# fritzsedlazeck/Sniffles

Hardware: AMD Instinct MI355X
Metric: SV-signatures clustered/sec (clustering + calling + QC + genotype + INS consensus) (higher is better)
Workload: dtype int32/f64

## Files before the change

sniffles_amd/csrc/snf_fused.h:

```cpp
#pragma once
#include "snf_stage_final.h"
#include "snf_stage_cluster.h"
#include "snf_stage_call.h"

namespace snf {

template <int K>
SNF_D void block_exscan256(const unsigned long long (&val)[K], unsigned long long (&excl)[K], unsigned long long (&tot)[K],
                           unsigned long long* lds) {
  const int tid = threadIdx.x, lane = tid & 63, wid = tid >> 6;
  unsigned long long incl[K];
#pragma unroll
  for (int k = 0; k < K; k++) {
    unsigned long long x = val[k];
#pragma unroll
    for (int d = 1; d < 64; d <<= 1) { const unsigned long long y = __shfl_up(x, d, 64); if (lane >= d) x += y; }
    incl[k] = x;
    if (lane == 63) lds[wid * K + k] = x;
  }
  __syncthreads();
#pragma unroll
  for (int k = 0; k < K; k++) {
    unsigned long long base = 0, all = 0;
#pragma unroll
// ... 119 lines not shown
  __global__ void __launch_bounds__(256) name(const View v, int64_t n) {      \
    __shared__ unsigned long long lds[8];                                     \
    const int64_t p = (int64_t)blockIdx.x * 256 + threadIdx.x;

__global__ void __launch_bounds__(256) z0_init(const View v, int64_t n) {
  const int64_t i = (int64_t)blockIdx.x * 256 + threadIdx.x;
  const int64_t T = v.T, G = 8 * T + 8;
  if (i < (int64_t)(sizeof(Counts) / 8)) {
    unsigned long long c0 = 0;
    if (v.win_ready && i == (int64_t)(offsetof(Counts, n_valid) / 8)) c0 = (unsigned long long)v.win_n_valid;
    if (v.win_ready && i == (int64_t)(offsetof(Counts, n_occ) / 8)) c0 = (unsigned long long)v.win_n_occ;
    ((unsigned long long*)v.cnt)[i] = c0;
  }
  if (i <= T) { v.t_cov_sum[i] = 0; v.t_status[i] = 0; }
  if (i <= T + 1) v.t_call_off[i] = 0;
  if (i < G) { v.grp_first_bin[i] = -1; v.grp_seed_lo[i] = -1; v.grp_seed_hi[i] = -1; v.grp_dirty[i] = 0; }
  if (i < TS_SLOTS * v.super_stride) v.tile_super[i] = 0;
  if (i < v.tile_stride) {
    v.tile_sums[(int64_t)TS_REFINED * v.tile_stride + i] = 0; v.tile_sums[(int64_t)TS_CALLS * v.tile_stride + i] = 0;
  }
  if (i == 0) *v.chain_epoch += 1u;
  if (v.wave_path && i < 3 * 64 * 16) v.big_cnt[i] = 0;
  if (v.wave_path && i < 3 * 64 * 16) v.d2cnt[i] = 0;
  if (i == 0 && v.NS > 0) {
    const int64_t N = v.NS;
    v.headflag[N] = 0; v.eligflag[N] = 0; v.fN[N] = 0; v.fL[N] = 0; v.runflag[N] = 0; v.clflag[N] = 0; v.rcflag[N] = 0; v.cdflag[N] = 0;
  }
}

SNF_FUSED_HEAD(a0k_keep)
  if (p < n) a0_keep_body(p, v);
  unsigned long long val[1] = {p < n ? (unsigned long long)v.pf_keep[p] : 0ull};
  tile_publish<1>(v, TS_KEEP, val, lds);
}
SNF_FUSED_HEAD(a0k_compact)
  unsigned long long val[1] = {p < n ? (unsigned long long)v.pf_keep[p] : 0ull}, off[1];
  tile_scan<1>(v, TS_KEEP, val, off, lds);
  if (p < n) {
    v.pf_scan[p] = (uint32_t)off[0];
    if (p == n - 1) v.cnt->n_kept = (int64_t)(off[0] + val[0]);
    a0_emit(p, v);
  }
}
SNF_FUSED_HEAD(a2k_heads)
  if (p < n) { a2_heads_body(p, v); v.rcflag[p] = 0; }
  unsigned long long val[1] = {p < n ? (unsigned long long)v.headflag[p] : 0ull};
// ... 201 lines not shown
```

sniffles_amd/csrc/snf_knobs.h:

```cpp
#pragma once
#include <climits>
#include <cstdlib>
#include <cstring>
#include <string>

namespace snf {

constexpr int KNOB_UNSET = INT_MIN;
inline bool env_set(const char* name) { return getenv(name) != nullptr; }
inline int env_int(const char* name, int unset) { const char* e = getenv(name); return e ? atoi(e) : unset; }
inline int env_pos(const char* name, int other) { const int v = env_int(name, 0); return v > 0 ? v : other; }
inline bool env_on(const char* name) { return env_int(name, 0) != 0; }
inline bool env_is(const char* name, const char* value) { const char* e = getenv(name); return e && strcmp(e, value) == 0; }
inline std::string env_str(const char* name) { const char* e = getenv(name); return e ? e : ""; }

struct BatchKnobs {
  bool wave_path = !env_set("SNF_NO_WAVE");
  bool fuse = !env_set("SNF_NO_FUSE");
  bool sort64 = env_set("SNF_SORT64");
  bool prefilter = !env_set("SNF_NO_PREFILTER");
  bool pf_spread = env_int("SNF_PF_SPREAD", 0) == 1;
  bool winfront = !env_set("SNF_NO_WINFRONT");
  int win_bits = env_int("SNF_WIN_BITS", 0);
  int win_bits_max = [] { const int v = env_int("SNF_WIN_BITS_MAX", 10); return v >= 6 && v <= 12 ? v : 10; }();
  bool w4_split = env_on("SNF_W4_SPLIT");
  bool pool_slices = !env_set("SNF_NO_POOL_SLICES");
  int fuse_copy = env_set("SNF_FUSE_COPY") ? env_on("SNF_FUSE_COPY") : -1;
  bool merge_reread = env_on("SNF_MERGE_REREAD");
  int run_gap = env_int("SNF_RUN_GAP", KNOB_UNSET);
  int chain = env_set("SNF_CHAIN") ? env_on("SNF_CHAIN") : env_set("SNF_NO_CHAIN") ? 0 : -1;
  int graph = env_set("SNF_GRAPH") ? env_on("SNF_GRAPH") : env_set("SNF_NO_GRAPH") ? 0 : -1;
  int heavy_n = env_int("SNF_HEAVY_N", 24);
  int e1_batch = env_int("SNF_E1_BATCH", 64);
  bool big_stage = !env_set("SNF_NO_BIG_STAGE");
  bool cov_exact = env_set("SNF_COV_EXACT");
  bool d4_thread = env_is("SNF_D4", "thread");
  bool d1_groups = !env_set("SNF_NO_D1_GROUPS");
  bool d2_groups = !env_set("SNF_NO_D2_GROUPS");
  bool d2_mid = env_set("SNF_D2_MID");
  bool rn_defer = !env_set("SNF_NO_RN_DEFER");
  bool rn_fuse = !env_set("SNF_NO_RN_FUSE");
  int grid_mult = env_int("SNF_GRID_MULT", 2);
  int grid_div = env_pos("SNF_GRID_DIV", 1);
  int occ_d2 = env_int("SNF_OCC_D2", 5);
  int occ_e1 = env_int("SNF_OCC_E1", 5);
  int occ_s = env_int("SNF_OCC_S", 5);
  int cons_nw = env_int("SNF_CONS_NW", 1);
  int cons_large_nw = env_int("SNF_CONS_LARGE_NW", 4);
  int cons_grid_mult = env_int("SNF_CONS_GRID_MULT", KNOB_UNSET);
  int cons_small_grid = env_pos("SNF_CONS_SMALL_GRID", 65536);
// ... 63 lines not shown
```

sniffles_amd/csrc/snf_lib.hip:

```cpp
#include "snf_stage_final.h"
#include "snf_wave_refine.h"
#include "snf_wave_cons.h"
#include "snf_fused.h"
#include "snf_stage_window.h"
#include "snf_stage_out.h"
#include "snf_wave_call.h"
#include "snf_wave_call_g.h"
#include "snf_wave_refine_g.h"
#include "snf_ctx.h"

#include <rocprim/device/device_radix_sort.hpp>
#include <rocprim/device/device_scan.hpp>

#include <fcntl.h>
#include <sys/file.h>
#include <unistd.h>

#include <atomic>
#include <map>
#include <tuple>
#include <cmath>
#include <ctime>
#include <memory>
#include <mutex>
// ... 887 lines not shown
    v.ws_seeds = dalloc<uint32_t>(b, nblk); v.ws_nf = dalloc<uint32_t>(b, nblk); v.ws_nl = dalloc<uint32_t>(b, nblk);
    v.whead = dalloc<uint64_t>(b, N1); v.whead2 = dalloc<uint64_t>(b, N1);
    dzero(b, v.wcnt, W1 * 4); dzero(b, v.wfill, W1 * 4);
  }
  uint32_t** u32s[] = {&v.headflag, &v.headscan, &v.eligflag, &v.eligscan, &v.fN, &v.pN, &v.fL, &v.pL, &v.runflag, &v.runscan,
                       &v.clflag, &v.clscan, &v.rcflag, &v.rcscan, &v.cdflag, &v.cdscan, &v.rnf, &v.rnp};
  for (auto pp : u32s) *pp = dalloc<uint32_t>(b, N1);
  v.seqnull = dalloc<uint8_t>(b, N); v.bin_lo = dalloc<int32_t>(b, N1); v.bin_key = dalloc<uint64_t>(b, N);
  v.bin_hap = dalloc<uint16_t>(b, 3 * (size_t)N); v.bin_elig = dalloc<uint8_t>(b, N);
  v.grp_first_bin = dalloc<int32_t>(b, 8 * (size_t)T + 8);
  v.L = dalloc<uint32_t>(b, N); v.LL = dalloc<uint32_t>(b, N); v.Lrec = dalloc<LeadRec>(b, N1); v.chdr = dalloc<ClusterHdr>(b, N1);
  int32_t** i32s[] = {&v.seed_bin, &v.seed_lo, &v.seed_hi, &v.seedL_lo, &v.seedL_hi, &v.seed_start, &v.seed_grp, &v.c_last, &v.c_end,
                      &v.nxt, &v.prv, &v.run_first, &v.run_last_head, &v.cl_head, &v.w0, &v.w1, &v.w2, &v.w3, &v.w4, &v.w5, &v.w6, &v.w7,
                      &v.F_orig, &v.F_svlen, &v.F_seq_len, &v.FI, &v.F_lpos, &v.rc_n_s, &v.rc_cl_s, &v.rc_lo, &v.rc_n, &v.rc_cluster};
  for (auto pp : i32s) *pp = dalloc<int32_t>(b, N1);
  double** f64s[] = {&v.s_mean0, &v.s_stdev0, &v.c_mean, &v.c_stdev, &v.run_b_stdev, &v.run_b_absmean};
  for (auto pp : f64s) *pp = dalloc<double>(b, N1);
  uint8_t** u8s[] = {&v.s_repeat0, &v.c_repeat, &v.run_b_repeat, &v.F_sel, &v.rc_keeplong_s, &v.rc_keeplong};
  for (auto pp : u8s) *pp = dalloc<uint8_t>(b, N1);
  v.c_ms = dalloc<ClusterSums>(b, N1);
  v.grp_dirty = dalloc<int32_t>(b, 8 * (size_t)T + 8); v.grp_seed_lo = dalloc<int32_t>(b, 8 * (size_t)T + 8);
  v.grp_seed_hi = dalloc<int32_t>(b, 8 * (size_t)T + 8);
  v.F_seq_off = dalloc<int64_t>(b, N1);
  v.fcopy = dalloc<FuseDesc>(b, N1); dzero(b, v.fcopy, N1 * sizeof(FuseDesc));
  v.cand = dalloc<snf_call_t>(b, N1); v.candx = dalloc<CallX>(b, N1);
  v.calls = dalloc<snf_call_t>(b, N1); v.callx = dalloc<CallX>(b, N1);
  v.rnames = dalloc<uint32_t>(b, 2 * (size_t)N + 1);
  const auto& lut = build_gt_lut(b->cfg);
  v.gt_lut = upload_vec(b, lut);
  v.cons_call = dalloc<int32_t>(b, N1);
  v.stripes = dalloc<unsigned long long>(b, 4 * 64 * 16);
  v.tile_stride = (int64_t)((N1 > (size_t)win_slots_max + 1 ? N1 : (size_t)win_slots_max + 1) / 256 + 2); v.tile_sums = dalloc<unsigned long long>(b, (size_t)v.tile_stride * TS_SLOTS);
  v.super_stride = v.tile_stride / 64 + 2; v.tile_super = dalloc<unsigned long long>(b, (size_t)v.super_stride * TS_SLOTS);
  v.chain_stride = v.tile_stride; v.chain = dalloc<unsigned long long>(b, (size_t)v.chain_stride * TS_SLOTS * 2);
  v.chain_ticket = dalloc<uint32_t>(b, TS_SLOTS + 2); v.chain_epoch = v.chain_ticket + TS_SLOTS;
  dzero(b, v.chain, (size_t)v.chain_stride * TS_SLOTS * 16); dzero(b, v.chain_ticket, (TS_SLOTS + 2) * 4);
  const bool small_batch = N <= 400000;
  v.chain_on = b->k.chain >= 0 ? b->k.chain : (small_batch ? 1 : 0);
  b->graph_mode = (b->k.graph >= 0 ? b->k.graph != 0 : small_batch) ? 2 : 0;
  v.fuse_defer = v.wave_path && (b->k.fuse_copy >= 0 ? b->k.fuse_copy != 0 : b->graph_mode == 0) ? 1 : 0;
  v.big_cap = (int64_t)(N1 / 64 + 2); v.big_cnt = dalloc<uint32_t>(b, 3 * 64 * 16); v.big_list = dalloc<int32_t>(b, (size_t)(3 * 64 * v.big_cap));
  v.big_wave = v.wave_path;
  { const int hn = b->k.heavy_n; v.heavy_n = hn > 8 && hn < 64 ? hn : 0; }
  v.d1_push = v.wave_path && b->k.d1_groups ? 1 : 0;
  v.d2_push = v.wave_path && b->k.d2_groups ? (b->k.d2_mid ? 2 : 1) : 0;
  { const int eb = b->k.e1_batch; v.e1_batch = (eb == 2 || eb == 4 || eb == 8 || eb == 16 || eb == 32) ? eb : 64; }
  v.stage_cap = b->k.big_stage ? 1 : 0;
// ... 287 lines not shown
  const int64_t n_blk = (N + 63) / 64;
  const bool split = b->k.w4_split && b->win_cap > 64 && b->h_n_big64 > 0 && b->h_n_big64 * 8 < n_blk;
  {
    Scope* sc = b->time_all ? new Scope(b, "w4s_segment", 0) : nullptr;
    if (split) {
      v.w4_mode = 1;
      hipLaunchKernelGGL(w4s_segment<64>, dim3((unsigned)n_blk), dim3(64), 0, b->cur, v, (int64_t)0);
      v.w4_mode = 2;
      if (b->win_cap == 256) hipLaunchKernelGGL(w4s_segment<256>, dim3((unsigned)b->h_n_big64), dim3(64), 0, b->cur, v, (int64_t)0);
      else hipLaunchKernelGGL(w4s_segment<SNF_WIN_MAXCAP>, dim3((unsigned)b->h_n_big64), dim3(64), 0, b->cur, v, (int64_t)0);
      v.w4_mode = 0;
    }
    else if (b->win_cap == 64) hipLaunchKernelGGL(w4s_segment<64>, dim3((unsigned)n_blk), dim3(64), 0, b->cur, v, (int64_t)0);
    else if (b->win_cap == 256) hipLaunchKernelGGL(w4s_segment<256>, dim3((unsigned)n_blk), dim3(64), 0, b->cur, v, (int64_t)0);
    else hipLaunchKernelGGL(w4s_segment<SNF_WIN_MAXCAP>, dim3((unsigned)n_blk), dim3(64), 0, b->cur, v, (int64_t)0);
    delete sc;
    SNF_HIP(hipGetLastError());
  }
  if (v.chain_on) CHAIN(w5c_offsets, n_blk);
  else { FUSED(w5a_sums, n_blk); FUSED(w5b_offsets, n_blk); }
  LAUNCH_Q(w6t_emit, v, N, 0);
}

void enqueue_fuse_copy(snf_batch_impl* b, hipEvent_t after) {
  View& v = b->v;
  if (!after) { SNF_HIP(hipEventRecord(b->ev_refined, b->stream)); after = b->ev_refined; }
  SNF_HIP(hipStreamWaitEvent(b->stream2, after, 0));
  hipStream_t prev = b->cur; b->cur = b->stream2;
  { Scope _s(b, "d1c_fusecopy", 0);
    int64_t grid = (v.NS + 63) / 64; if (grid > 2048) grid = 2048;
    hipLaunchKernelGGL(d1c_fusecopy, dim3((unsigned)grid), dim3(64), 0, b->cur, v, (int64_t)0);
    SNF_HIP(hipGetLastError()); }
  b->cur = prev;
  SNF_HIP(hipEventRecord(b->ev_fcopy, b->stream2));
  b->fcopy_open = true;
}

void run_call_candidates(snf_batch_impl* b) {
  SNF_TRACE("snf_batch_call_candidates (enqueue)");
  b->pass_idle = false;
  View& v = b->v;
  int T = v.T;
  const int64_t N = v.NS;
  b->reads_ready = true; b->cov_avg_ready = true; b->finalized = false;
  begin_pass_timing(b);
  pass_begins(b);
  join_open_candidates(b);
  b->chain_slot = -1;
  if (process_knobs().chain_gate && !b->capturing) {
    DevicePacing& P = pacing_of(b);
    std::lock_guard<std::mutex> g(P.pace_mu);
    const unsigned long long my = P.chain_seq++;
    hipEvent_t& mine = P.chain_ev[my & 1]; hipEvent_t prev = P.chain_ev[(my + 1) & 1];
    if (!mine) SNF_HIP(hipEventCreateWithFlags(&mine, hipEventDisableTiming));
    b->chain_slot = (int)(my & 1);
    if (prev && P.passes_in_flight.load() > 1) SNF_HIP(hipStreamWaitEvent(b->stream, prev, 0));
  }
  v.rn_defer = ((v.out_mode & SNF_OUT_EXECUTE) && !v.cfg.no_qc && b->k.rn_defer && b->k.fuse && N <= ((int64_t)1 << 25)) ? 1 : 0;
  b->rn_state = v.rn_defer ? 1 : 0;
  if (b->k.timeline) SNF_HIP(hipEventRecord(b->ev_base, b->stream));
  enqueue_pass_init(b);
  if (v.wave_path && !b->fused) dzero(b, v.big_cnt, sizeof(uint32_t) * 3 * 64 * 16);
  if (v.wave_path && !b->fused) dzero(b, v.d2cnt, sizeof(uint32_t) * 3 * 64 * 16);
  b->finalize_runs = 0;
  fork_mark(b);
  if (b->k.readprep == 0) enqueue_read_prep(b);
  const bool front = v.front && b->fused && N > 0;
  if (front) enqueue_window_front(b); else enqueue_keys(b);
  if (N > 0) {
    if (!b->fused) {
      uint32_t* tails[] = {v.headflag, v.eligflag, v.fN, v.fL, v.runflag, v.clflag, v.rcflag, v.cdflag};
      for (auto p : tails) dzero(b, p + N, sizeof(uint32_t));
    }
    if (!front) {
    if (v.key32) prim_sort_pairs<uint32_t>(b, (uint32_t*)v.key_in, (uint32_t*)v.key_out, v.val_in, v.val_out, N, v.key_nbits + 1, "sort_lead_keys");
    else prim_sort_pairs<uint64_t>(b, v.key_in, v.key_out, v.val_in, v.val_out, N, v.key_nbits + 1, "sort_lead_keys");
    }
    if (b->fused) {
    if (!front) {
    FUSED(a2k_heads, N);
    FUSED(a3k_bins, N);
    { Scope _s(b, "a4_binstats", N * 16); FUSED(a4k_binstats, N); }
    FUSED(a5k_leadflags, N);
    { Scope _s(b, "a6_scatter", N * 16); FUSED(a6k_scatter, N); }
    FUSED(a7k_seeds, N);
    }
// ... 478 lines not shown
  if (ok) ok = hipGraphInstantiate(&exec, graph, nullptr, nullptr, 0) == hipSuccess && exec != nullptr;
  if (!ok) {
    (void)hipGetLastError();
    if (graph) (void)hipGraphDestroy(graph);
    b->graph_failed = true;
    if (v.prof) fprintf(stderr, "[SNF_PROF] pass graph: capture failed, passes stay eager\n");
    run_call_candidates(b); run_finalize(b);
    return;
  }
  g.graph = graph; g.exec = exec; g.rn_state = b->rn_state; g.rn_defer = v.rn_defer; g.cap_out = b->hb_out.cap; g.cap_alt = b->hb_alt.cap;
  if (v.prof) { size_t nn = 0; (void)hipGraphGetNodes(graph, nullptr, &nn); fprintf(stderr, "[SNF_PROF] pass graph: captured (%zu nodes)\n", nn); }
  SNF_HIP(hipGraphLaunch(g.exec, b->stream));
}
void destroy_graphs(snf_batch_impl* b) {
  for (auto& kv : b->graphs) { if (kv.second.exec) (void)hipGraphExecDestroy(kv.second.exec); if (kv.second.graph) (void)hipGraphDestroy(kv.second.graph); }
  b->graphs.clear();
}

void collect_timings(snf_batch_impl* b) {
  b->timings.clear();
#ifdef SNF_ITRACE
  if (b->k.prof && b->v.itrace) {
    static const char* nm[SNF_IT_SLOTS] = {"w1_hist", "w3_scatter", "w4s_segment", "w6t_emit", "d1g_refine", "d1w_refine", "d2g_call", "d2w_call", "e3b_offsets",
                                           "e1w_finalize", "cons SMALL", "cons LARGE", "d4s_coverage", "f4w_emit", "cons ROWS", ""};
    std::vector<uint32_t> h((size_t)SNF_IT_SLOTS * SNF_IT_CAP * 2);
    (void)hipMemcpy(h.data(), b->v.itrace, h.size() * 4, hipMemcpyDeviceToHost);
    (void)hipMemset(b->v.itrace, 0, h.size() * 4);
    for (int k = 0; k < SNF_IT_SLOTS; k++) {
      struct E { uint32_t t0, dur, wg; };
      std::vector<E> es;
      for (int64_t i = 0; i < SNF_IT_CAP; i++) { const uint32_t* o = &h[2 * ((size_t)k * SNF_IT_CAP + i)]; if (o[1] & 0x80000000u) es.push_back({o[0], o[1] & 0x7fffffffu, (uint32_t)i}); }
      if (es.empty()) continue;
      uint32_t base = es[0].t0;
      for (auto& e : es) if ((int32_t)(e.t0 - base) < 0) base = e.t0;
      uint32_t span = 0; double sum = 0;
      for (auto& e : es) { e.t0 -= base; span = std::max(span, e.t0 + e.dur); sum += e.dur; }
      std::vector<uint32_t> d; for (auto& e : es) d.push_back(e.dur);
      std::sort(d.begin(), d.end());
      auto pc = [&](double q) { return d[(size_t)(q * (d.size() - 1))] * 0.01; };
      fprintf(stderr, "[SNF_ITRACE] %-13s %6zu workgroups, span %7.1f us, sum %9.1f us = %6.0f in flight on average; duration us p50 %.1f p90 %.1f p99 %.1f max %.1f; in flight at 12 points:",
              nm[k], es.size(), span * 0.01, sum * 0.01, sum / (span ? span : 1), pc(0.5), pc(0.9), pc(0.99), pc(1.0));
      for (int q = 0; q < 12; q++) { const uint32_t t = (uint32_t)((uint64_t)span * (2 * q + 1) / 24); int act = 0; for (auto& e : es) act += e.t0 <= t && t < e.t0 + e.dur; fprintf(stderr, " %d", act); }
      std::sort(es.begin(), es.end(), [](const E& a, const E& c) { return a.t0 + a.dur > c.t0 + c.dur; });
      fprintf(stderr, "; last to end:");
      for (size_t q = 0; q < es.size() && q < 4; q++) fprintf(stderr, " wg %u +%.1f for %.1f", es[q].wg, es[q].t0 * 0.01, es[q].dur * 0.01);
      fprintf(stderr, "\n");
    }
// ... 86 lines not shown

bool settle_alt_stage(snf_batch_impl* b) {
  View& v = b->v;
  if (!v.wave_path || !b->fused || v.NS <= 0) return false;
  const Counts& c = *b->h_cnt;
  if (c.n_cls[7] == 0 && c.n_cons_fallback == 0) return false;
  run_alt_fallback(b);
  LAUNCH_Q(z1_results, v, tail_threads(v), 0);
  dsync(b);
  return true;
}

void do_fetch(snf_batch_impl* b, int stage, snf_result_t* out) {
  SNF_TRACE(stage >= 1 ? "snf_batch_fetch(1): wait + result block" : "snf_batch_fetch(0): wait + candidates");
  View& v = b->v;
  int T = v.T;
  b->r_status.assign(T, 0); b->r_off.assign(T + 1, 0); b->r_cov.assign(T, NAN);
  full_sync(b);
  pass_waited(b);
  if (b->h_cnt->overflow) fail(b->h_cnt->overflow & 2 ? "internal: hand-over list of the call kernels overflowed" : "internal: fused-sequence pool overflow");
  if (v.prof) {
    const Counts& c = *b->h_cnt;
    fprintf(stderr, "[SNF_PROF] counts: valid %lld windows %lld bins %lld seeds %lld clusters %lld refined %lld calls %lld | cons calls %lld reads %lld "
                    "fallback %lld alt bytes %lld fused bytes through the shared counter %llu (the rest in the waves' own slices; the split depends on scheduling, the total and the capacity do not) | ALT lists copy %llu small %llu large %llu/%llu/%llu/%llu thread %llu rows %llu\n", (long long)c.n_valid, (long long)c.n_occ, (long long)c.n_bins, (long long)c.n_seeds, (long long)c.n_clusters,
            (long long)c.n_rc, (long long)c.n_calls, (long long)c.n_cons, (long long)c.n_cons_reads, (long long)c.n_cons_fallback,
            (long long)c.alt_total, c.pool_extra_used, c.n_cls[0], c.n_cls[1], c.n_cls[2], c.n_cls[3], c.n_cls[4], c.n_cls[5], c.n_cls[6], c.n_cls[7]);
  }
  memcpy(b->r_status.data(), v.res_status, (size_t)T * sizeof(int32_t));
  memcpy(b->r_cov.data(), v.res_cov, (size_t)T * sizeof(double));
  if (stage >= 1 && b->finalized) {
    const bool alt_late = settle_alt_stage(b);
    {
      const Counts& c = *b->h_cnt;
      bool skipped_work = false;
      for (int k = 0; k < 3; k++) {
        if (b->skipped_big[k] && c.n_big[k] > 0) skipped_work = true;
        b->hist_big[k] = c.n_big[k];
      }
      if (skipped_work) { b->pass_idle = true; fail("internal: a pass skipped x_big although items were handed to it (the handle's next pass launches it)"); }
      b->have_big_hist = true;
      b->hist_small = (int64_t)c.n_cls[1]; b->hist_large = (int64_t)(c.n_cls[2] + c.n_cls[3] + c.n_cls[4] + c.n_cls[5]); b->hist_copy = (int64_t)c.n_cls[0];
      b->hist_calls = c.n_calls; b->have_hist = true;
    }
    const OutHdr h = *v.res_out;
    const uint8_t* base = (const uint8_t*)b->hb_out.p;
    const int64_t alt_total_now = b->h_cnt->alt_total;
    const bool block_there = !h.in_pinned && b->staged_kernel && b->stage_block_copied && v.stage_out_pin == (uint8_t*)b->hb_out.p && h.bytes <= v.stage_out_cap;
    const bool alt_there = !b->h_cnt->alt_in_pinned && b->staged_kernel && b->stage_alt_copied && !alt_late && v.stage_alt_pin == (uint8_t*)b->hb_alt.p && alt_total_now <= v.stage_alt_cap;
    bool need_sync = false;
// ... 805 lines not shown
```

sniffles_amd/csrc/snf_view.h:

```cpp
#pragma once
#include "../../include/sniffles_amd.h"
#include "snf_rt.h"

namespace snf {

struct Counts {
  int64_t n_valid, n_bins, n_seeds, NF, NLL, n_runs, n_clusters, n_rc, n_calls;
  int64_t n_ins_calls, alt_total, n_cons, tab_total, aln_total, n_cons_reads, rn_total;
  int64_t n_dirty_groups;
  int64_t n_kept;
  int64_t n_big[3];
  int64_t n_occ;
  int64_t max_win;
  int64_t n_big64;
  unsigned long long n_w4big;
  int64_t n_cons_fallback;
  unsigned long long cons_bytes[4];
  unsigned long long n_cls[8];
  unsigned long long pool_extra_used;
#ifdef SNF_CONS_PROFILE
  unsigned long long dbg[32];
#endif
#ifdef SNF_C1_PROFILE
  unsigned long long c1p[16];
#endif
  int32_t overflow;
  int32_t alt_in_pinned;
};

struct GtEntry {
  int8_t order0;
  int8_t gq;
  int8_t z;
  int8_t _pad;
// ... 161 lines not shown
  OutHdr* out_hdr;
  OutHdr* res_out;
  uint8_t* out_dev; int64_t out_dev_cap;
  uint8_t* out_pin; int64_t out_pin_cap;
  Counts* res_cnt; int32_t* res_status; int64_t* res_off; double* res_cov;
  int64_t* res_rn_total;
  uint32_t *rnf, *rnp;

  int32_t *seed_bin, *seed_lo, *seed_hi, *seedL_lo, *seedL_hi, *seed_start, *seed_grp;
  double *s_mean0, *s_stdev0; uint8_t* s_repeat0;
  double *c_mean, *c_stdev; uint8_t* c_repeat;
  int32_t *c_last, *c_end, *nxt, *prv;
  ClusterSums* c_ms;
  int32_t *run_first;
  int32_t *run_last_head;
  double *run_b_stdev, *run_b_absmean; uint8_t* run_b_repeat;
  int32_t* grp_dirty;
  int32_t *grp_seed_lo, *grp_seed_hi;

  int32_t* cl_head;
  int32_t *w0, *w1, *w2, *w3, *w4, *w5, *w6;
  int32_t *F_orig, *F_svlen, *F_seq_len; int64_t* F_seq_off; uint8_t* F_sel; int32_t* FI;
  int32_t* F_lpos;
  FuseDesc* fcopy; int32_t fuse_defer, _pad_fd;
  int32_t *rc_n_s, *rc_cl_s; uint8_t* rc_keeplong_s;
  int32_t *rc_lo, *rc_n, *rc_cluster; uint8_t* rc_keeplong;
  snf_call_t* cand; CallX* candx;
  snf_call_t* calls; CallX* callx;
  uint32_t* rnames;

  const GtEntry* gt_lut;
  int32_t* cons_call;
  int64_t *cons_tab_off, *cons_aln_off, *cons_read_off, *cons_tab_sz;
  int64_t *sz_tab, *sz_aln, *sz_rd;
  int64_t *sc_tab, *sc_aln, *sc_rd;
  uint64_t* tab_key; int32_t* tab_pos; uint8_t* tab_state; int64_t tab_cap;
  uint8_t* aln; int64_t aln_cap;
  uint8_t* aln_kept;
  int32_t *cr_call, *cr_read;
  uint8_t* alt_pool; int64_t alt_cap;
  uint8_t* alt_pin; int64_t alt_pin_cap;
  uint8_t* stage_out_pin; int64_t stage_out_cap; uint8_t* stage_alt_pin; int64_t stage_alt_cap;
  unsigned long long* stripes;
  unsigned long long* tile_super; int64_t super_stride;
  unsigned long long* chain; int64_t chain_stride; uint32_t* chain_ticket; uint32_t* chain_epoch; int32_t chain_on, _pad_chain;
  unsigned long long* tile_sums; int64_t tile_stride;
  ConsDesc* cdesc;
// ... 41 lines not shown
```

sniffles_amd/csrc/snf_wave_refine.h:

```cpp
#pragma once
#include "snf_stage_call.h"

namespace snf {

#define SNF_WAVE 64

SNF_D uint64_t wave_bcast_u64(uint64_t x, int src) {
  uint32_t lo = __builtin_amdgcn_readlane((uint32_t)x, src), hi = __builtin_amdgcn_readlane((uint32_t)(x >> 32), src);
  return ((uint64_t)hi << 32) | lo;
}
SNF_D int32_t wave_bcast_i32(int32_t x, int src) { return (int32_t)__builtin_amdgcn_readlane((uint32_t)x, src); }

#define SNF_DPP_STEPS(STEP) STEP(0x111, 0xf) STEP(0x112, 0xf) STEP(0x114, 0xf) STEP(0x118, 0xf) STEP(0x142, 0xa) STEP(0x143, 0xc)
SNF_D int32_t wave_incl_scan(int32_t x, int lane) {
  (void)lane;
#define SNF_STEP(ctrl, rows) x += __builtin_amdgcn_update_dpp(0, x, ctrl, rows, 0xf, false);
  SNF_DPP_STEPS(SNF_STEP)
#undef SNF_STEP
  return x;
}
SNF_D int64_t wave_incl_scan64(int64_t x, int lane) {
  (void)lane;
#define SNF_STEP(ctrl, rows) { const uint32_t lo_ = (uint32_t)__builtin_amdgcn_update_dpp(0, (int)(uint32_t)(uint64_t)x, ctrl, rows, 0xf, false), \
                                              hi_ = (uint32_t)__builtin_amdgcn_update_dpp(0, (int)(uint32_t)((uint64_t)x >> 32), ctrl, rows, 0xf, false); \
// ... 36 lines not shown
    for (int k = 0; k < 4; k++) {
      so[k] = __shfl(p_src, z[k], SNF_WAVE); dt[k] = __shfl(p_dst, z[k], SNF_WAVE);
      const int32_t l = __shfl(p_len, z[k], SNF_WAVE);
      sl[k] = k < np ? l : 0;
    }
#pragma unroll
    for (int k = 0; k < 4; k++) {
      const int32_t nfull = sl[k] & ~15;
      buf[k] = make_uint4(0, 0, 0, 0); tb[k] = 0;
      if (lane * 16 < nfull) buf[k] = *(const u128_any*)(v.pool + so[k] + lane * 16);
      if (nfull + lane < sl[k]) tb[k] = v.pool[so[k] + nfull + lane];
    }
#pragma unroll
    for (int k = 0; k < 4; k++) {
      const int32_t nfull = sl[k] & ~15;
      if (lane * 16 < nfull) *(u128_any*)(v.pool + dt[k] + lane * 16) = buf[k];
      if (nfull + lane < sl[k]) v.pool[dt[k] + nfull + lane] = tb[k];
      for (int32_t bb = SNF_WAVE * 16 + lane * 16; bb < nfull; bb += SNF_WAVE * 16)
        *(u128_any*)(v.pool + dt[k] + bb) = *(const u128_any*)(v.pool + so[k] + bb);
    }
  }
}

template <bool DEFER>
SNF_D void fuse_parts(const View& v, int lane, int64_t slot, bool p_act, int64_t p_src, int32_t p_len, int64_t p_dst) {
  if constexpr (DEFER) { if (p_act && p_len > 0) v.fcopy[slot] = FuseDesc::make(p_src, p_len, p_dst); }
  else wave_copy_parts(v, lane, p_act, p_src, p_len, p_dst);
}

__global__ void __launch_bounds__(SNF_WAVE) d1c_fusecopy(const View v, int64_t n_unused) {
  const int lane = threadIdx.x;
  int64_t n = v.cnt->NF; if (n > v.N) n = v.N;
  for (int64_t base = (int64_t)blockIdx.x * SNF_WAVE; base < n; base += (int64_t)gridDim.x * SNF_WAVE) {
    const int64_t s = base + lane;
    FuseDesc d{0, 0};
    if (s < n) d = v.fcopy[s];
    const int32_t len = d.len();
    if (__ballot(len != 0) == 0ull) continue;
    if (len != 0) v.fcopy[s] = FuseDesc{0, 0};
    const bool on = len > 0 && d.src() + len <= v.pool_cap && d.dst() + len <= v.pool_cap;
    wave_copy_parts(v, lane, on, d.src(), on ? len : 0, d.dst());
  }
}

SNF_D int64_t d1list_prefix(const View& v, int lane, int32_t* pre) {
  int32_t cnt = (int32_t)v.d2cnt[(2 * 64 + lane) * 16];
  if (cnt > (int32_t)v.d2cap) cnt = (int32_t)v.d2cap;
  const int32_t inc = wave_incl_scan(cnt, lane);
  if (lane == 0) pre[0] = 0;
  pre[lane + 1] = inc;
  __syncthreads();
  return pre[64];
}
SNF_D int32_t d1list_at(const View& v, int64_t i, const int32_t* pre) {
  int lo = 0, hi = 63;
  while (lo < hi) { const int mid = (lo + hi + 1) >> 1; if (pre[mid] <= (int32_t)i) lo = mid; else hi = mid - 1; }
  return v.d2_list[2][(int64_t)lo * v.d2cap + (i - pre[lo])];
}

struct WaveLds {
  int32_t perm[SNF_WAVE];
  int32_t seg_start[SNF_WAVE];
  int32_t seg_key[SNF_WAVE];
};

#define SNF_PERMUTE_SETUP(rank_, active_)         \
  __syncthreads();                                \
  if (active_) lds.perm[rank_] = lane;            \
  __syncthreads();                                \
  const int src_ = lds.perm[lane < n_ ? lane : 0];
#define SNF_GATHER(x) __shfl((x), src_, SNF_WAVE)

#ifdef SNF_CONS_PROFILE
#define SNF_RT_DECL unsigned long long rt_acc[6] = {0, 0, 0, 0, 0, 0}; unsigned long long rt_t = __builtin_amdgcn_s_memtime();
#define SNF_RT(k) do { const unsigned long long rt_n = __builtin_amdgcn_s_memtime(); rt_acc[k] += rt_n - rt_t; rt_t = rt_n; } while (0)
#define SNF_RT_FLUSH() do { if (lane == 0) for (int pk = 0; pk < 6; pk++) atomicAdd(&v.cnt->dbg[24 + pk], rt_acc[pk]); } while (0)
#else
#define SNF_RT_DECL
#define SNF_RT(k) do { } while (0)
#define SNF_RT_FLUSH() do { } while (0)
#endif
template <bool DEFER>
__global__ void __launch_bounds__(SNF_WAVE) d1w_refine(const View v, int64_t n_unused) {
  IT_SCOPE(5)
  __shared__ WaveLds lds;
  const int lane = threadIdx.x;
  const snf_config_t& cfg = v.cfg;
  __shared__ int32_t d1pre[65];
  const bool from_list = v.d1_from_list != 0;
  const int64_t n_clusters = from_list ? d1list_prefix(v, lane, d1pre) : v.cnt->n_clusters;
  auto CL = [&](int64_t it) -> int64_t { return from_list ? (int64_t)d1list_at(v, it, d1pre) : it; };
  const int64_t stride = gridDim.x;
  int64_t c_cur = blockIdx.x < n_clusters ? CL(blockIdx.x) : 0, c_nxt = blockIdx.x + stride < n_clusters ? CL(blockIdx.x + stride) : 0;
  ClusterHdr hd_cur = blockIdx.x < n_clusters ? v.chdr[c_cur] : ClusterHdr{};
  ClusterHdr hd_nxt = blockIdx.x + stride < n_clusters ? v.chdr[c_nxt] : ClusterHdr{};
  LeadRec rec_cur{};
  if (lane < hd_cur.n && hd_cur.n <= SNF_WAVE) rec_cur = v.Lrec[hd_cur.lo + lane];
  SNF_RT_DECL
  int64_t slice_used = from_list ? (v.pool_slice >> 1) : 0;
  for (int64_t it = blockIdx.x; it < n_clusters; it += stride) {
    SNF_RT(5);
    const ClusterHdr hd = hd_cur; const LeadRec rec = rec_cur;
    const int64_t c = c_cur;
    hd_cur = hd_nxt; c_cur = c_nxt;
    if (it + stride < n_clusters && lane < hd_cur.n && hd_cur.n <= SNF_WAVE) rec_cur = v.Lrec[hd_cur.lo + lane];
    if (it + 2 * stride < n_clusters) { c_nxt = CL(it + 2 * stride); hd_nxt = v.chdr[c_nxt]; }
// ... 62 lines not shown
      SNF_RT(2);
      int64_t new_off = 0; bool need_copy = start && seq_ok && nparts > 1;
      if (__ballot(need_copy)) {
        const int64_t mine = need_copy ? tot_seq : 0;
        const int64_t incl = wave_incl_scan64(mine, lane);
        const int64_t wave_total = __shfl(incl, 63, SNF_WAVE);
        int64_t base;
        if (slice_used + wave_total <= v.pool_slice) {
          base = v.pool_len + (int64_t)blockIdx.x * v.pool_slice + slice_used;
          slice_used += wave_total;
        } else {
          int64_t got = 0;
          if (lane == 0) got = (int64_t)atomicAdd(&v.cnt->pool_extra_used, (unsigned long long)wave_total);
          base = v.pool_extra_base + __shfl(got, 0, SNF_WAVE);
        }
        new_off = base + (incl - mine);
        if (need_copy && new_off + tot_seq > v.pool_cap) { atomicOr(&v.cnt->overflow, 1); need_copy = false; }
      }
      {
        const unsigned long long upto = lane == 63 ? ~0ull : ((2ull << lane) - 1ull);
        const int my_start = (act && (smask & upto)) ? 63 - __builtin_clzll(smask & upto) : 0;
        const bool p_act = act && __shfl((int)need_copy, my_start, SNF_WAVE) != 0;
        const int64_t p_dst = __shfl(new_off, my_start, SNF_WAVE) + (x_seq - __shfl(x_seq, my_start, SNF_WAVE));
        fuse_parts<DEFER>(v, lane, (int64_t)lo + lane, p_act, s_seq_off, p_act ? s_seq_len : 0, p_dst);
      }
      const bool ok_seq = start && seq_ok && (nparts == 1 || need_copy);
      m = __builtin_popcountll(smask);
      const int kidx = __builtin_popcountll(smask & ((1ull << lane) - 1ull));
      __syncthreads();
      if (start) lds.perm[kidx] = lane;
      __syncthreads();
      const int src2 = lds.perm[lane < m ? lane : 0];
      f_orig = (int32_t)__shfl(s_o, src2, SNF_WAVE); f_lp = __shfl(s_lp, src2, SNF_WAVE);
      f_svlen = (int32_t)__shfl(tot_svlen, src2, SNF_WAVE);
      const int32_t t_seq_len = ok_seq ? (nparts == 1 ? s_seq_len : (int32_t)tot_seq) : -1;
      const int64_t t_seq_off = ok_seq ? (nparts == 1 ? s_seq_off : new_off) : 0;
      f_seq_len = __shfl(t_seq_len, src2, SNF_WAVE);
      f_seq_off = __shfl(t_seq_off, src2, SNF_WAVE);
      }
    }
    SNF_RT(3);
    const bool fact = lane < m;
    if (fact) {
      v.F_orig[lo + lane] = f_orig; v.F_svlen[lo + lane] = f_svlen; v.F_lpos[lo + lane] = lo + f_lp;
      v.F_seq_len[lo + lane] = f_seq_len; v.F_seq_off[lo + lane] = f_seq_off;
    }

// ... 99 lines not shown
```

sniffles_amd/csrc/snf_wave_refine_g.h:

```cpp
#pragma once
#include "snf_wave_call_g.h"

namespace snf {

template <int G> SNF_D int64_t gscan64(int64_t x, int gl) {
#pragma unroll
  for (int d = 1; d < G; d <<= 1) { const int64_t y = __shfl_up(x, d, SNF_WAVE); if (gl >= d) x += y; }
  return x;
}
template <int G> SNF_D int32_t gscan32(int32_t x, int gl) {
#pragma unroll
  for (int d = 1; d < G; d <<= 1) { const int32_t y = __shfl_up(x, d, SNF_WAVE); if (gl >= d) x += y; }
  return x;
}
template <int G> SNF_D int64_t gshfl_i64(int64_t x, int src, int gbase) { return (int64_t)gshfl_u64<G>((uint64_t)x, src, gbase); }

struct GroupLds { int32_t perm[SNF_WAVE], seg_start[SNF_WAVE], seg_key[SNF_WAVE]; };

template <int G, bool DEFER>
__global__ void __launch_bounds__(SNF_WAVE) d1g_refine(const View v, int64_t n_unused) {
  IT_SCOPE(4)
  static_assert(G == 8, "group width in use");
  constexpr int NG = SNF_WAVE / G;
  __shared__ GroupLds lds;
// ... 82 lines not shown
      const bool seq_ok = (e_has - x_has) == nparts;
      int64_t new_off = 0; bool need_copy = start && seq_ok && nparts > 1;
      if (__ballot(need_copy)) {
        const int64_t mine = need_copy ? tot_seq : 0;
        const int64_t incl = wave_incl_scan64(mine, lane);
        const int64_t wave_total = __shfl(incl, 63, SNF_WAVE);
        int64_t pbase;
        if (slice_used + wave_total <= (v.pool_slice >> 1)) {
          pbase = v.pool_len + (int64_t)blockIdx.x * v.pool_slice + slice_used;
          slice_used += wave_total;
        } else {
          int64_t got = 0;
          if (lane == 0) got = (int64_t)atomicAdd(&v.cnt->pool_extra_used, (unsigned long long)wave_total);
          pbase = v.pool_extra_base + __shfl(got, 0, SNF_WAVE);
        }
        new_off = pbase + (incl - mine);
        if (need_copy && new_off + tot_seq > v.pool_cap) { atomicOr(&v.cnt->overflow, 1); need_copy = false; }
      }
      {
        const unsigned long long upto = (2ull << gl) - 1ull;
        const int my_start = (fact0 && (smask & upto)) ? 63 - __builtin_clzll(smask & upto) : 0;
        const bool p_act = fact0 && __shfl((int)need_copy, gbase + my_start, SNF_WAVE) != 0;
        const int64_t p_dst = __shfl(new_off, gbase + my_start, SNF_WAVE) + (x_seq - __shfl(x_seq, gbase + my_start, SNF_WAVE));
        fuse_parts<DEFER>(v, lane, (int64_t)lo + gl, p_act, s_seq_off, p_act ? s_seq_len : 0, p_dst);
      }
      const bool ok_seq = start && seq_ok && (nparts == 1 || need_copy);
      const int mm = __builtin_popcountll(smask);
      const int kidx = __builtin_popcountll(smask & ((1ull << gl) - 1ull));
      __syncthreads();
      if (start) lds.perm[gbase + kidx] = gl;
      __syncthreads();
      const int src2 = gbase + (fuse ? lds.perm[gbase + (gl < mm ? gl : 0)] : gl);
      const int32_t t_seq_len = ok_seq ? (nparts == 1 ? s_seq_len : (int32_t)tot_seq) : -1;
      const int64_t t_seq_off = ok_seq ? (nparts == 1 ? s_seq_off : new_off) : 0;
      const int32_t g_orig = (int32_t)__shfl(s_o, src2, SNF_WAVE), g_lp = __shfl(s_lp, src2, SNF_WAVE);
      const int32_t g_svlen = (int32_t)__shfl(tot_svlen, src2, SNF_WAVE);
      const int32_t g_seq_len = __shfl(t_seq_len, src2, SNF_WAVE);
      const int64_t g_seq_off = __shfl(t_seq_off, src2, SNF_WAVE);
      if (fuse) { m = mm; f_orig = g_orig; f_lp = g_lp; f_svlen = g_svlen; f_seq_len = g_seq_len; f_seq_off = g_seq_off; }
      __syncthreads();
    }
    const bool fact = gl < m;
    if (fact) {
      v.F_orig[lo + gl] = f_orig; v.F_svlen[lo + gl] = f_svlen; v.F_lpos[lo + gl] = lo + f_lp;
      v.F_seq_len[lo + gl] = f_seq_len; v.F_seq_off[lo + gl] = f_seq_off;
    }
    bool done = !valid;
// ... 122 lines not shown
```

Before: 3.843 billion.

## Compact deferred fuse-copy descriptors into per-stripe lists and copy four per wave

Deferred fuse-copy descriptors are no longer written into a sparse per-signature array. Each wave now appends them, via a wave-aggregated atomic, into one of 64 striped compact lists, and copies in place when a list overflows. The copy kernel now runs on a fixed grid, walks only the populated entries, and handles four descriptors per wave with 16-byte vector loads. This removes the full-length scan and re-zeroing of the sparse array. In exchange it adds atomics, extra counters to zero each pass, and a host-side join of the previous fuse copy before each pass; d1w_refine also gets an occupancy hint.

Result: slower. 3.790 billion (-1.4%).

```diff
diff --git a/sniffles_amd/csrc/snf_fused.h b/sniffles_amd/csrc/snf_fused.h
--- a/sniffles_amd/csrc/snf_fused.h
+++ b/sniffles_amd/csrc/snf_fused.h
@@ -165,6 +165,7 @@
   if (i == 0) *v.chain_epoch += 1u;
   if (v.wave_path && i < 3 * 64 * 16) v.big_cnt[i] = 0;
   if (v.wave_path && i < 3 * 64 * 16) v.d2cnt[i] = 0;
+  if (v.wave_path && i < 64 * 16) v.fcnt[i] = 0;
   if (i == 0 && v.NS > 0) {
     const int64_t N = v.NS;
     v.headflag[N] = 0; v.eligflag[N] = 0; v.fN[N] = 0; v.fL[N] = 0; v.runflag[N] = 0; v.clflag[N] = 0; v.rcflag[N] = 0; v.cdflag[N] = 0;
diff --git a/sniffles_amd/csrc/snf_knobs.h b/sniffles_amd/csrc/snf_knobs.h
--- a/sniffles_amd/csrc/snf_knobs.h
+++ b/sniffles_amd/csrc/snf_knobs.h
@@ -26,6 +26,7 @@
   bool w4_split = env_on("SNF_W4_SPLIT");
   bool pool_slices = !env_set("SNF_NO_POOL_SLICES");
   int fuse_copy = env_set("SNF_FUSE_COPY") ? env_on("SNF_FUSE_COPY") : -1;
+  int fuse_list_cap = env_int("SNF_FUSE_LIST_CAP", -1);
   bool merge_reread = env_on("SNF_MERGE_REREAD");
   int run_gap = env_int("SNF_RUN_GAP", KNOB_UNSET);
   int chain = env_set("SNF_CHAIN") ? env_on("SNF_CHAIN") : env_set("SNF_NO_CHAIN") ? 0 : -1;
diff --git a/sniffles_amd/csrc/snf_lib.hip b/sniffles_amd/csrc/snf_lib.hip
--- a/sniffles_amd/csrc/snf_lib.hip
+++ b/sniffles_amd/csrc/snf_lib.hip
@@ -933,7 +933,16 @@
   v.grp_dirty = dalloc<int32_t>(b, 8 * (size_t)T + 8); v.grp_seed_lo = dalloc<int32_t>(b, 8 * (size_t)T + 8);
   v.grp_seed_hi = dalloc<int32_t>(b, 8 * (size_t)T + 8);
   v.F_seq_off = dalloc<int64_t>(b, N1);
-  v.fcopy = dalloc<FuseDesc>(b, N1); dzero(b, v.fcopy, N1 * sizeof(FuseDesc));
+#ifdef SNF_FCOPY_PARENT_LAYOUT
+  if (N1 >= ((size_t)1 << 20)) {
+    const int64_t per = (int64_t)((N1 - 256) / 64);
+    v.fcopy = dalloc<FuseDesc>(b, N1); v.fcnt = (uint32_t*)(v.fcopy + (N1 - 256));
+    v.fcap = b->k.fuse_list_cap >= 0 && b->k.fuse_list_cap < per ? b->k.fuse_list_cap : per;
+  } else
+#endif
+  { const int64_t per = (int64_t)((N1 + 63) / 64) + 128;
+    v.fcopy = dalloc<FuseDesc>(b, (size_t)(64 * per)); v.fcnt = dalloc<uint32_t>(b, 64 * 16);
+    v.fcap = b->k.fuse_list_cap >= 0 && b->k.fuse_list_cap < per ? b->k.fuse_list_cap : per; }
   v.cand = dalloc<snf_call_t>(b, N1); v.candx = dalloc<CallX>(b, N1);
   v.calls = dalloc<snf_call_t>(b, N1); v.callx = dalloc<CallX>(b, N1);
   v.rnames = dalloc<uint32_t>(b, 2 * (size_t)N + 1);
@@ -1267,14 +1276,16 @@
   LAUNCH_Q(w6t_emit, v, N, 0);
 }
 
+#ifndef SNF_FCOPY_GRID
+#define SNF_FCOPY_GRID 512
+#endif
 void enqueue_fuse_copy(snf_batch_impl* b, hipEvent_t after) {
   View& v = b->v;
   if (!after) { SNF_HIP(hipEventRecord(b->ev_refined, b->stream)); after = b->ev_refined; }
   SNF_HIP(hipStreamWaitEvent(b->stream2, after, 0));
   hipStream_t prev = b->cur; b->cur = b->stream2;
   { Scope _s(b, "d1c_fusecopy", 0);
-    int64_t grid = (v.NS + 63) / 64; if (grid > 2048) grid = 2048;
-    hipLaunchKernelGGL(d1c_fusecopy, dim3((unsigned)grid), dim3(64), 0, b->cur, v, (int64_t)0);
+    hipLaunchKernelGGL(d1c_fusecopy, dim3(SNF_FCOPY_GRID), dim3(64), 0, b->cur, v, (int64_t)0);
     SNF_HIP(hipGetLastError()); }
   b->cur = prev;
   SNF_HIP(hipEventRecord(b->ev_fcopy, b->stream2));
@@ -1291,6 +1302,7 @@
   begin_pass_timing(b);
   pass_begins(b);
   join_open_candidates(b);
+  if (!b->capturing) join_fuse_copy(b);
   b->chain_slot = -1;
   if (process_knobs().chain_gate && !b->capturing) {
     DevicePacing& P = pacing_of(b);
@@ -1307,6 +1319,7 @@
   enqueue_pass_init(b);
   if (v.wave_path && !b->fused) dzero(b, v.big_cnt, sizeof(uint32_t) * 3 * 64 * 16);
   if (v.wave_path && !b->fused) dzero(b, v.d2cnt, sizeof(uint32_t) * 3 * 64 * 16);
+  if (v.wave_path && !b->fused) dzero(b, v.fcnt, sizeof(uint32_t) * 64 * 16);
   b->finalize_runs = 0;
   fork_mark(b);
   if (b->k.readprep == 0) enqueue_read_prep(b);
@@ -1831,7 +1844,7 @@
 #ifdef SNF_ITRACE
   if (b->k.prof && b->v.itrace) {
     static const char* nm[SNF_IT_SLOTS] = {"w1_hist", "w3_scatter", "w4s_segment", "w6t_emit", "d1g_refine", "d1w_refine", "d2g_call", "d2w_call", "e3b_offsets",
-                                           "e1w_finalize", "cons SMALL", "cons LARGE", "d4s_coverage", "f4w_emit", "cons ROWS", ""};
+                                           "e1w_finalize", "cons SMALL", "cons LARGE", "d4s_coverage", "f4w_emit", "cons ROWS", "d1c_fusecopy"};
     std::vector<uint32_t> h((size_t)SNF_IT_SLOTS * SNF_IT_CAP * 2);
     (void)hipMemcpy(h.data(), b->v.itrace, h.size() * 4, hipMemcpyDeviceToHost);
     (void)hipMemset(b->v.itrace, 0, h.size() * 4);
@@ -1964,9 +1977,10 @@
   if (v.prof) {
     const Counts& c = *b->h_cnt;
     fprintf(stderr, "[SNF_PROF] counts: valid %lld windows %lld bins %lld seeds %lld clusters %lld refined %lld calls %lld | cons calls %lld reads %lld "
-                    "fallback %lld alt bytes %lld fused bytes through the shared counter %llu (the rest in the waves' own slices; the split depends on scheduling, the total and the capacity do not) | ALT lists copy %llu small %llu large %llu/%llu/%llu/%llu thread %llu rows %llu\n", (long long)c.n_valid, (long long)c.n_occ, (long long)c.n_bins, (long long)c.n_seeds, (long long)c.n_clusters,
+                    "fallback %lld alt bytes %lld fused bytes through the shared counter %llu (the rest in the waves' own slices; the split depends on scheduling, the total and the capacity do not) "
+                    "fused parts appended %lld in place %lld | ALT lists copy %llu small %llu large %llu/%llu/%llu/%llu thread %llu rows %llu\n", (long long)c.n_valid, (long long)c.n_occ, (long long)c.n_bins, (long long)c.n_seeds, (long long)c.n_clusters,
             (long long)c.n_rc, (long long)c.n_calls, (long long)c.n_cons, (long long)c.n_cons_reads, (long long)c.n_cons_fallback,
-            (long long)c.alt_total, c.pool_extra_used, c.n_cls[0], c.n_cls[1], c.n_cls[2], c.n_cls[3], c.n_cls[4], c.n_cls[5], c.n_cls[6], c.n_cls[7]);
+            (long long)c.alt_total, c.pool_extra_used, (long long)c.n_fuse[0], (long long)c.n_fuse[1], c.n_cls[0], c.n_cls[1], c.n_cls[2], c.n_cls[3], c.n_cls[4], c.n_cls[5], c.n_cls[6], c.n_cls[7]);
   }
   memcpy(b->r_status.data(), v.res_status, (size_t)T * sizeof(int32_t));
   memcpy(b->r_cov.data(), v.res_cov, (size_t)T * sizeof(double));
diff --git a/sniffles_amd/csrc/snf_view.h b/sniffles_amd/csrc/snf_view.h
--- a/sniffles_amd/csrc/snf_view.h
+++ b/sniffles_amd/csrc/snf_view.h
@@ -10,6 +10,7 @@
   int64_t n_dirty_groups;
   int64_t n_kept;
   int64_t n_big[3];
+  int64_t n_fuse[2];
   int64_t n_occ;
   int64_t max_win;
   int64_t n_big64;
@@ -217,7 +218,7 @@
   int32_t *w0, *w1, *w2, *w3, *w4, *w5, *w6;
   int32_t *F_orig, *F_svlen, *F_seq_len; int64_t* F_seq_off; uint8_t* F_sel; int32_t* FI;
   int32_t* F_lpos;
-  FuseDesc* fcopy; int32_t fuse_defer, _pad_fd;
+  FuseDesc* fcopy; uint32_t* fcnt; int64_t fcap; int32_t fuse_defer, _pad_fd;
   int32_t *rc_n_s, *rc_cl_s; uint8_t* rc_keeplong_s;
   int32_t *rc_lo, *rc_n, *rc_cluster; uint8_t* rc_keeplong;
   snf_call_t* cand; CallX* candx;
diff --git a/sniffles_amd/csrc/snf_wave_refine.h b/sniffles_amd/csrc/snf_wave_refine.h
--- a/sniffles_amd/csrc/snf_wave_refine.h
+++ b/sniffles_amd/csrc/snf_wave_refine.h
@@ -82,40 +82,101 @@
   }
 }
 
-template <bool DEFER>
-SNF_D void fuse_parts(const View& v, int lane, int64_t slot, bool p_act, int64_t p_src, int32_t p_len, int64_t p_dst) {
-  if constexpr (DEFER) { if (p_act && p_len > 0) v.fcopy[slot] = FuseDesc::make(p_src, p_len, p_dst); }
-  else wave_copy_parts(v, lane, p_act, p_src, p_len, p_dst);
-}
-
-__global__ void __launch_bounds__(SNF_WAVE) d1c_fusecopy(const View v, int64_t n_unused) {
-  const int lane = threadIdx.x;
-  int64_t n = v.cnt->NF; if (n > v.N) n = v.N;
-  for (int64_t base = (int64_t)blockIdx.x * SNF_WAVE; base < n; base += (int64_t)gridDim.x * SNF_WAVE) {
-    const int64_t s = base + lane;
-    FuseDesc d{0, 0};
-    if (s < n) d = v.fcopy[s];
-    const int32_t len = d.len();
-    if (__ballot(len != 0) == 0ull) continue;
-    if (len != 0) v.fcopy[s] = FuseDesc{0, 0};
-    const bool on = len > 0 && d.src() + len <= v.pool_cap && d.dst() + len <= v.pool_cap;
-    wave_copy_parts(v, lane, on, d.src(), on ? len : 0, d.dst());
-  }
-}
-
-SNF_D int64_t d1list_prefix(const View& v, int lane, int32_t* pre) {
-  int32_t cnt = (int32_t)v.d2cnt[(2 * 64 + lane) * 16];
-  if (cnt > (int32_t)v.d2cap) cnt = (int32_t)v.d2cap;
-  const int32_t inc = wave_incl_scan(cnt, lane);
+SNF_D int64_t stripes_prefix(int32_t items, int lane, int32_t* pre) {
+  const int32_t inc = wave_incl_scan(items, lane);
   if (lane == 0) pre[0] = 0;
   pre[lane + 1] = inc;
   __syncthreads();
   return pre[64];
 }
-SNF_D int32_t d1list_at(const View& v, int64_t i, const int32_t* pre) {
+SNF_D int stripe_of(int64_t i, const int32_t* pre) {
   int lo = 0, hi = 63;
   while (lo < hi) { const int mid = (lo + hi + 1) >> 1; if (pre[mid] <= (int32_t)i) lo = mid; else hi = mid - 1; }
-  return v.d2_list[2][(int64_t)lo * v.d2cap + (i - pre[lo])];
+  return lo;
+}
+
+SNF_D int64_t d1list_prefix(const View& v, int lane, int32_t* pre) {
+  int32_t cnt = (int32_t)v.d2cnt[(2 * 64 + lane) * 16];
+  if (cnt > (int32_t)v.d2cap) cnt = (int32_t)v.d2cap;
+  return stripes_prefix(cnt, lane, pre);
+}
+SNF_D int32_t d1list_at(const View& v, int64_t i, const int32_t* pre) {
+  const int s = stripe_of(i, pre);
+  return v.d2_list[2][(int64_t)s * v.d2cap + (i - pre[s])];
+}
+
+SNF_D void wave_copy_rest(const View& v, int lane, bool on, int64_t p_src, int32_t p_len, int64_t p_dst) {
+  typedef uint32_t __attribute__((aligned(1))) u32_any;
+  for (unsigned long long pm = __ballot(on); pm; pm &= pm - 1ull) {
+    const int z = __builtin_ctzll(pm);
+    const int64_t so = (int64_t)wave_bcast_u64((uint64_t)p_src, z), dt = (int64_t)wave_bcast_u64((uint64_t)p_dst, z);
+    const int32_t sl = wave_bcast_i32(p_len, z), nfull = sl & ~3;
+    for (int32_t bb = lane * 4; bb < nfull; bb += SNF_WAVE * 4) *(u32_any*)(v.pool + dt + bb) = *(const u32_any*)(v.pool + so + bb);
+    if (nfull + lane < sl) v.pool[dt + nfull + lane] = v.pool[so + nfull + lane];
+  }
+}
+template <bool DEFER>
+SNF_D void fuse_parts(const View& v, int lane, bool p_act, int64_t p_src, int32_t p_len, int64_t p_dst) {
+  if constexpr (DEFER) {
+    const bool has = p_act && p_len > 0;
+    const unsigned long long pm = __ballot(has);
+    if (pm == 0ull) return;
+    const int np = __builtin_popcountll(pm), leader = __builtin_ctzll(pm), st = (int)(blockIdx.x & 63);
+    uint32_t at = 0;
+    if (lane == leader) at = atomicAdd(&v.fcnt[st * 16], (uint32_t)np);
+    at = (uint32_t)__shfl((int32_t)at, leader, SNF_WAVE);
+    const uint32_t e = at + (uint32_t)__builtin_popcountll(pm & ((1ull << lane) - 1ull));
+    const bool put = has && (int64_t)e < v.fcap;
+    if (put) v.fcopy[(int64_t)st * v.fcap + e] = FuseDesc::make(p_src, p_len, p_dst);
+    if ((int64_t)at + np > v.fcap) wave_copy_rest(v, lane, has && !put, p_src, p_len, p_dst);
+  }
+  else wave_copy_parts(v, lane, p_act, p_src, p_len, p_dst);
+}
+
+__global__ void __launch_bounds__(SNF_WAVE) d1c_fusecopy(const View v, int64_t n_unused) {
+  IT_SCOPE(15)
+  typedef uint4 __attribute__((aligned(1))) u128_any;
+  __shared__ int32_t pre[65], nent[SNF_WAVE];
+  const int lane = threadIdx.x;
+  {
+    const int64_t c_all = (int64_t)v.fcnt[lane * 16], c_list = c_all > v.fcap ? v.fcap : c_all;
+    nent[lane] = (int32_t)c_list;
+    if (blockIdx.x == 0) {
+      const int64_t in_list = wave_last64(wave_incl_scan64(c_list, lane)), in_place = wave_last64(wave_incl_scan64(c_all - c_list, lane));
+      if (lane == 0) { v.cnt->n_fuse[0] = in_list; v.cnt->n_fuse[1] = in_place; }
+    }
+  }
+  const int64_t n_groups = stripes_prefix((nent[lane] + 3) >> 2, lane, pre);
+  const int32_t off = lane * 16;
+  for (int64_t g = blockIdx.x; g < n_groups; g += gridDim.x) {
+    const int s = __builtin_amdgcn_readfirstlane(stripe_of(g, pre));
+    const int32_t e0 = __builtin_amdgcn_readfirstlane((int32_t)(g - pre[s]) * 4), ne = __builtin_amdgcn_readfirstlane(nent[s]);
+    const FuseDesc* list = v.fcopy + (int64_t)s * v.fcap;
+    int64_t so[4], dt[4]; int32_t sl[4], nf[4], maxfull = 0;
+#pragma unroll
+    for (int k = 0; k < 4; k++) {
+      FuseDesc d{0, 0};
+      if (e0 + k < ne) d = list[e0 + k];
+      d.a = wave_bcast_u64(d.a, 0); d.b = wave_bcast_u64(d.b, 0);
+      const int32_t len = d.len();
+      so[k] = d.src(); dt[k] = d.dst();
+      sl[k] = (len > 0 && so[k] + len <= v.pool_cap && dt[k] + len <= v.pool_cap) ? len : 0;
+      nf[k] = sl[k] & ~15;
+      maxfull = nf[k] > maxfull ? nf[k] : maxfull;
+    }
+    uint8_t tb[4];
+#pragma unroll
+    for (int k = 0; k < 4; k++) { tb[k] = 0; if (nf[k] + lane < sl[k]) tb[k] = v.pool[so[k] + nf[k] + lane]; }
+    for (int32_t base = 0; base < maxfull; base += SNF_WAVE * 16) {
+      uint4 buf[4];
+#pragma unroll
+      for (int k = 0; k < 4; k++) { buf[k] = make_uint4(0, 0, 0, 0); if (base + off < nf[k]) buf[k] = *(const u128_any*)(v.pool + (so[k] + base) + off); }
+#pragma unroll
+      for (int k = 0; k < 4; k++) if (base + off < nf[k]) *(u128_any*)(v.pool + (dt[k] + base) + off) = buf[k];
+    }
+#pragma unroll
+    for (int k = 0; k < 4; k++) if (nf[k] + lane < sl[k]) v.pool[dt[k] + nf[k] + lane] = tb[k];
+  }
 }
 
 struct WaveLds {
@@ -141,7 +202,7 @@
 #define SNF_RT_FLUSH() do { } while (0)
 #endif
 template <bool DEFER>
-__global__ void __launch_bounds__(SNF_WAVE) d1w_refine(const View v, int64_t n_unused) {
+__global__ void __launch_bounds__(SNF_WAVE, DEFER ? 6 : 1) d1w_refine(const View v, int64_t n_unused) {
   IT_SCOPE(5)
   __shared__ WaveLds lds;
   const int lane = threadIdx.x;
@@ -250,7 +311,7 @@
         const int my_start = (act && (smask & upto)) ? 63 - __builtin_clzll(smask & upto) : 0;
         const bool p_act = act && __shfl((int)need_copy, my_start, SNF_WAVE) != 0;
         const int64_t p_dst = __shfl(new_off, my_start, SNF_WAVE) + (x_seq - __shfl(x_seq, my_start, SNF_WAVE));
-        fuse_parts<DEFER>(v, lane, (int64_t)lo + lane, p_act, s_seq_off, p_act ? s_seq_len : 0, p_dst);
+        fuse_parts<DEFER>(v, lane, p_act, s_seq_off, p_act ? s_seq_len : 0, p_dst);
       }
       const bool ok_seq = start && seq_ok && (nparts == 1 || need_copy);
       m = __builtin_popcountll(smask);
diff --git a/sniffles_amd/csrc/snf_wave_refine_g.h b/sniffles_amd/csrc/snf_wave_refine_g.h
--- a/sniffles_amd/csrc/snf_wave_refine_g.h
+++ b/sniffles_amd/csrc/snf_wave_refine_g.h
@@ -128,7 +128,7 @@
         const int my_start = (fact0 && (smask & upto)) ? 63 - __builtin_clzll(smask & upto) : 0;
         const bool p_act = fact0 && __shfl((int)need_copy, gbase + my_start, SNF_WAVE) != 0;
         const int64_t p_dst = __shfl(new_off, gbase + my_start, SNF_WAVE) + (x_seq - __shfl(x_seq, gbase + my_start, SNF_WAVE));
-        fuse_parts<DEFER>(v, lane, (int64_t)lo + gl, p_act, s_seq_off, p_act ? s_seq_len : 0, p_dst);
+        fuse_parts<DEFER>(v, lane, p_act, s_seq_off, p_act ? s_seq_len : 0, p_dst);
       }
       const bool ok_seq = start && seq_ok && (nparts == 1 || need_copy);
       const int mm = __builtin_popcountll(smask);
```
